# lipku/LiveTalking

Measured on NVIDIA H100. Metric: lip-sync frames/sec (wav2lip256, 256x256, batch 16, mel + U-Net fwd + paste-back), higher is better.
Workload: dtype f16 (fp32 accumulate); mel f64; paste u8

## Files before the change

livetalking_b200/csrc/conv_halo.cu:

```cuda
#include <cuda.h>

#include <atomic>
#include <mutex>
#include <utility>

#include "conv_halo.h"
#include "ltb_internal.h"
#include "ptx_sm90.cuh"

#ifdef LTB_HALO_DIAG
#include <cstdlib>
#define LTB_DIAG(bit) (p.dbg & (bit))
#else
#define LTB_DIAG(bit) 0
#endif

namespace ltb {

constexpr int kHaloP = 10;
constexpr int kHaloThreads = 384;
constexpr int kProducerRegs = 40, kConsumerRegs = 232;
constexpr int kSms = 132;

template <int BN, int NSUB, int NACC, int TAPS, int RC = 0>
struct HaloCfg {
  static constexpr bool HALO = (TAPS != 1);
  static constexpr bool S2 = (TAPS == 10);
  static constexpr int P = S2 ? 9 : (HALO ? kHaloP : 8);
  static constexpr int HR = S2 ? 16 * NSUB + 1 : (HALO ? 16 * NSUB + 2 : 16 * NSUB);
  static constexpr int TG = (TAPS == 9 || TAPS == 10) ? 3 : (TAPS == 16 ? 4 : 1);
  static constexpr int PLANE_BYTES = (HR * P * 128 + 1023) & ~1023;
  static constexpr int A_BYTES_RAW = (S2 ? 4 : 1) * HR * P * 128;
  static constexpr int A_BYTES = S2 ? 4 * PLANE_BYTES : ((A_BYTES_RAW + 1023) & ~1023);
  static constexpr int B_BYTES = TG * BN * 128;
  static constexpr int BUDGET = 223 * 1024;
  static constexpr int A_STAGES_STREAM = S2 ? 2 : ((BN <= 32) ? 4 : (BN <= 64 ? 3 : (NSUB == 1 ? 3 : 2)));
  static constexpr int A_STAGES_RES = ((BUDGET - RC * TG * B_BYTES) / A_BYTES) > 4 ? 4 : ((BUDGET - RC * TG * B_BYTES) / A_BYTES);
  static constexpr int A_STAGES = RC ? A_STAGES_RES : A_STAGES_STREAM;
  static constexpr bool RES_PREFETCH = (BN == 128 && NSUB == 2 && NACC == 1 && TAPS == 9 && RC == 0);
  static constexpr int RES_BYTES = RES_PREFETCH ? 128 * BN * 2 : 0;
  static constexpr int B_STAGES_MAX = (BUDGET - A_STAGES * A_BYTES - RES_BYTES) / B_BYTES;
  static constexpr int B_STAGES = RC ? RC * TG : (B_STAGES_MAX > 8 ? 8 : B_STAGES_MAX);
  static constexpr bool LAG = RC || B_STAGES >= 2 * TG;
  static constexpr int ACOLS = NACC * BN;
  static constexpr int SMEM_BYTES = A_STAGES * A_BYTES + B_STAGES * B_BYTES + RES_BYTES + 1024;
  static_assert(NSUB * ACOLS <= 256, "register accumulator overflow");
  static_assert(B_STAGES >= 2, "not enough shared memory for the weight ring");
  static_assert(A_STAGES >= 2, "not enough shared memory for the halo ring");
  static_assert(SMEM_BYTES + 3584 <= 227 * 1024, "shared memory overflow (dynamic + static)");
};

struct SubpixelView {
  int stage, view, slot0, brow, nslots;
};
constexpr int subpixel_view(int vy, int vx) { return (vy + 1) * kHaloP + (vx + 1); }
template <int TAPS>
struct SubpixelTable;
template <>
struct SubpixelTable<9> {
  static constexpr int NV = 5;
  static constexpr SubpixelView v[NV] = {{0, 0, 0, 0, 3}, {1, 1, 1, 0, 2}, {1, kHaloP + 1, 2, 2, 1}, {2, 0, 3, 2, 1}, {2, kHaloP, 2, 0, 2}};
};
template <>
struct SubpixelTable<16> {
  static constexpr int NV = 10;
  static constexpr SubpixelView v[NV] = {{0, subpixel_view(0, 0), 0, 0, 4},
                                         {1, subpixel_view(-1, 0), 0, 0, 2},  {1, subpixel_view(0, 1), 1, 2, 2},
                                         {2, subpixel_view(1, 0), 2, 0, 2},   {2, subpixel_view(0, -1), 0, 2, 1}, {2, subpixel_view(0, -1), 3, 3, 1},
                                         {3, subpixel_view(-1, -1), 0, 0, 1}, {3, subpixel_view(-1, 1), 1, 1, 1}, {3, subpixel_view(1, 1), 2, 2, 1},
                                         {3, subpixel_view(1, -1), 3, 3, 1}};
};

template <int BN, int SLOT0, int BROW, int R, size_t... S>
__device__ __forceinline__ void subpixel_slots(float (&acc)[R], uint64_t a, uint32_t b_lo, uint32_t b_hi, std::index_sequence<S...>) {
  (wgmma_ss_at<BN, (SLOT0 + (int)S) * BN>(acc, a, wgmma_lohi(b_lo + (BROW + (uint32_t)S) * BN * 8u, b_hi), 1u), ...);
}

template <int BN, int TAPS, int R, size_t... V>
__device__ __forceinline__ void subpixel_issue(float (&acc)[R], int j, int k, uint32_t a_lo0, uint32_t b_lo0, uint32_t a_hi, uint32_t b_hi,
                                               std::index_sequence<V...>) {
  (
      [&] {
        constexpr SubpixelView g = SubpixelTable<TAPS>::v[V];
        if (j == g.stage)
          subpixel_slots<BN, g.slot0, g.brow>(acc, wgmma_lohi(a_lo0 + g.view * 8u + k * 2u, a_hi), b_lo0 + k * 2u, b_hi,
                                              std::make_index_sequence<g.nslots>{});
      }(),
      ...);
}

__device__ __forceinline__ void quad_transpose(uint32_t (&x)[4], int lane) {
  const bool b2 = lane & 2, b1 = lane & 1;
  uint32_t s0 = __shfl_xor_sync(0xffffffffu, b2 ? x[0] : x[2], 2);
  uint32_t s1 = __shfl_xor_sync(0xffffffffu, b2 ? x[1] : x[3], 2);
  x[0] = b2 ? s0 : x[0];
  x[1] = b2 ? s1 : x[1];
  x[2] = b2 ? x[2] : s0;
  x[3] = b2 ? x[3] : s1;
  s0 = __shfl_xor_sync(0xffffffffu, b1 ? x[0] : x[1], 1);
  s1 = __shfl_xor_sync(0xffffffffu, b1 ? x[2] : x[3], 1);
  x[0] = b1 ? s0 : x[0];
  x[2] = b1 ? s1 : x[2];
  x[1] = b1 ? x[1] : s0;
  x[3] = b1 ? x[3] : s1;
}

constexpr bool halo_res_smem_ok(int BN, int NSUB, int NACC, int TAPS) { return TAPS == 9 && NACC == 1 && BN * NSUB <= 128; }

template <int BN, int NSUB, int NACC, int TAPS, int RC, bool GRP>
__global__ void __launch_bounds__(kHaloThreads, 1) conv_halo_wgmma_kernel(const __grid_constant__ HaloParams p) {
  static_assert(!GRP || TAPS == 1, "grouped weights exist in GEMM mode only");
  using C = HaloCfg<BN, NSUB, NACC, TAPS, RC>;
  extern __shared__ uint8_t smem_raw[];
  __shared__ __align__(8) uint64_t a_full[C::A_STAGES], a_empty[C::A_STAGES];
  __shared__ __align__(8) uint64_t b_full[C::B_STAGES], b_empty[C::B_STAGES];
  __shared__ float head_sw[100];
  constexpr int kGnSmem = (NACC == 1) ? 512 : 1;
  __shared__ float gn_acc[kGnSmem];

  const int tid = threadIdx.x, warp = tid >> 5, lane = tid & 31;
  constexpr bool kHeadOk = (BN == 32 && NACC == 1 && TAPS == 9);
  const bool gn_smem = NACC == 1 && p.gn_stats != nullptr && p.gn_images * p.gn_groups * 2 <= kGnSmem;
  if (gn_smem)
    for (int i = tid; i < p.gn_images * p.gn_groups * 2; i += kHaloThreads) gn_acc[i] = 0.f;
  constexpr bool kHaloMode = C::HALO;
  if (kHeadOk && p.head_out && tid < 99) head_sw[tid] = (tid < 96) ? p.head_w[tid] : p.head_b[tid - 96];
  const uint32_t smem0 = (smem_u32(smem_raw) + 1023u) & ~1023u;
  const uint32_t a_smem = smem0;
  const uint32_t b_smem = smem0 + C::A_STAGES * C::A_BYTES;
  const int chunks = (p.Cin + 63) / 64;

  if (tid == 0) {
    for (int s = 0; s < C::A_STAGES; ++s) {
      mbar_init(smem_u32(&a_full[s]), 1);
      mbar_init(smem_u32(&a_empty[s]), 8);
    }
    for (int s = 0; s < C::B_STAGES; ++s) {
      mbar_init(smem_u32(&b_full[s]), 1);
      mbar_init(smem_u32(&b_empty[s]), 8);
    }
    mbar_fence_init();
    tma_prefetch_desc(&p.tm_in);
    tma_prefetch_desc(&p.tm_w);
  }
  __syncthreads();

  const int tiles_m = kHaloMode ? p.tiles_x * p.tiles_y * p.N : p.tiles_x;

  pdl_launch_dependents();
  if (RC && warp == 8 && lane == 0) {
    mbar_arrive_expect_tx(smem_u32(&b_full[0]), RC * C::TG * C::B_BYTES);
    for (int c = 0; c < RC; ++c)
      for (int j = 0; j < C::TG; ++j)
        tma_load_3d(b_smem + (c * C::TG + j) * C::B_BYTES, &p.tm_w, smem_u32(&b_full[0]), c * 64, 0, j * C::TG);
  }
  pdl_wait();

  if (warp >= 8) {
    setmaxnreg_dec<kProducerRegs>();
    if (warp == 8 && lane == 0) {
      uint32_t ai = 0, bi = 0;
      for (int t = blockIdx.x; t < p.total_tiles; t += gridDim.x) {
        const int nt = t / tiles_m;
        int mt = t - nt * tiles_m;
        int img = 0, y0 = 0, x0 = 0;
        int g_row = 0, g_slot = 0;
        if constexpr (GRP) {
          const int g = mt / p.group_tiles;
          g_row = g * p.group_rows + (mt - g * p.group_tiles) * (128 * NSUB);
          g_slot = p.group_slot[g];
        }
        if (kHaloMode) {
          img = mt / (p.tiles_x * p.tiles_y);
          mt -= img * (p.tiles_x * p.tiles_y);
          const int ty = mt / p.tiles_x, tx = mt - ty * p.tiles_x;
          y0 = ty * (16 * NSUB) + p.halo_y0;
          x0 = tx * 8 + p.halo_x0;
        }
        for (int c = 0; c < chunks; ++c) {
          const uint32_t as = ai % C::A_STAGES;
          mbar_wait(smem_u32(&a_empty[as]), ((ai / C::A_STAGES) & 1u) ^ 1u);
          if (LTB_DIAG(8)) {
            mbar_arrive(smem_u32(&a_full[as]));
          } else {
            mbar_arrive_expect_tx(smem_u32(&a_full[as]), C::A_BYTES_RAW);
            if (C::S2) {
#pragma unroll
              for (int pl = 0; pl < 4; ++pl)
                tma_load_4d(a_smem + as * C::A_BYTES + pl * C::PLANE_BYTES, &p.tm_in, smem_u32(&a_full[as]), c * 64,
                            2 * (x0 + 1) - (pl & 1), 2 * (y0 + 1) - (pl >> 1), img);
            } else if (kHaloMode) tma_load_4d(a_smem + as * C::A_BYTES, &p.tm_in, smem_u32(&a_full[as]), c * 64, x0, y0, img);
            else if constexpr (GRP) tma_load_2d(a_smem + as * C::A_BYTES, &p.tm_in, smem_u32(&a_full[as]), c * 64, g_row);
            else tma_load_2d(a_smem + as * C::A_BYTES, &p.tm_in, smem_u32(&a_full[as]), c * 64, mt * (128 * NSUB));
          }
          ++ai;
          if (RC) continue;
          for (int j = 0; j < C::TG; ++j) {
            const uint32_t bs = bi % C::B_STAGES;
            mbar_wait(smem_u32(&b_empty[bs]), ((bi / C::B_STAGES) & 1u) ^ 1u);
            if (LTB_DIAG(16)) {
              mbar_arrive(smem_u32(&b_full[bs]));
              ++bi;
              continue;
            }
            mbar_arrive_expect_tx(smem_u32(&b_full[bs]), C::B_BYTES);
            if (kHaloMode) tma_load_3d(b_smem + bs * C::B_BYTES, &p.tm_w, smem_u32(&b_full[bs]), c * 64, nt * BN, j * C::TG);
            else if constexpr (GRP) tma_load_3d(b_smem + bs * C::B_BYTES, &p.tm_w, smem_u32(&b_full[bs]), c * 64, nt * BN, g_slot);
            else tma_load_2d(b_smem + bs * C::B_BYTES, &p.tm_w, smem_u32(&b_full[bs]), c * 64, nt * BN);
            ++bi;
          }
        }
      }
    }
  } else {
    setmaxnreg_inc<kConsumerRegs>();
    const int wg = warp >> 2, wq = warp & 3;
    const int cq = 2 * (lane & 3);
    constexpr uint32_t kAHi = wgmma_hi_128b(C::P * 128);
    constexpr uint32_t kBHi = wgmma_hi_128b(1024);
    constexpr uint32_t kRowsPerSub = C::HALO ? 16u * C::P : 128u;
    const uint32_t wg_off = (uint32_t)wg * (C::HALO ? 8u * C::P : 64u) * 8u;
    constexpr bool kResHalo = halo_res_smem_ok(BN, NSUB, NACC, TAPS);
    const int res_row = (8 * wg + 2 * wq + ((lane >> 3) & 1) + 1) * C::P + (lane & 7) + 1;
    const int res_kb = lane >> 4;
    auto halo_pix = [&](int img, int ty, int tx, int sub, int sl, int r, bool& ok) -> size_t {
      const int gy = ty * (16 * NSUB) + sub * 16 + wg * 8 + (r >> 3), gx = tx * 8 + (r & 7);
      ok = gy < p.GH && gx < p.GW;
      return ((size_t)img * p.OH + gy * p.osy + p.acc_oy[sl]) * p.OW + gx * p.osx + p.acc_ox[sl];
    };
    const uint32_t res_buf = b_smem + C::B_STAGES * C::B_BYTES;
    if (RC) mbar_wait(smem_u32(&b_full[0]), 0);
    uint32_t ai = 0, bi = 0;
    for (int t = blockIdx.x; t < p.total_tiles; t += gridDim.x) {
      const int nt = t / tiles_m;
      int mt = t - nt * tiles_m;
      int img = 0, ty = 0, tx = 0;
      if (kHaloMode) {
        img = mt / (p.tiles_x * p.tiles_y);
        mt -= img * (p.tiles_x * p.tiles_y);
        ty = mt / p.tiles_x;
        tx = mt - ty * p.tiles_x;
      }
      const int n0 = nt * BN;
      const bool res_pf = C::RES_PREFETCH && p.res != nullptr && !LTB_DIAG(1);
      auto res_src = [&](int sub, int r, bool& ok) {
        const size_t px = halo_pix(img, ty, tx, sub, 0, r, ok);
        return reinterpret_cast<const uint4*>(p.res + (ok ? px : 0) * p.RCtot + p.rc_off + n0 + 8 * (lane & 3));
      };
      if constexpr (C::RES_PREFETCH) {
        if (res_pf) {
#pragma unroll
          for (int hh = 0; hh < 2; ++hh) {
            bool ok;
            const uint4* src = res_src(0, wq * 16 + (lane >> 2) + 8 * hh, ok);
#pragma unroll
            for (int m = 0; m < BN / 32; ++m) cp_async16(res_buf + ((hh * (BN / 32) + m) * 256 + tid) * 16, src + 4 * m, ok ? 16u : 0u);
          }
          cp_async_commit();
        }
      }
      uint4 rpf[2][BN / 32];
      float acc[NSUB][C::ACOLS / 2];
#pragma unroll
      for (int s = 0; s < NSUB; ++s)
#pragma unroll
        for (int i = 0; i < C::ACOLS / 2; ++i) acc[s][i] = 0.f;
      uint32_t rh[NSUB][2][BN / 8];
      const int n0_res = (t / tiles_m) * BN;
      const int c_res = (kResHalo && p.res_halo) ? n0_res / 64 : chunks;
      const int cb_res = (BN == 32) ? (n0_res & 63) >> 3 : 0;
      uint32_t pend_as = 0, pend_bs = 0;
      bool pend = false;
#pragma unroll 1
      for (int c = 0; c < chunks; ++c) {
        const uint32_t as = ai % C::A_STAGES;
        mbar_wait(smem_u32(&a_full[as]), (ai / C::A_STAGES) & 1u);
        if constexpr (kResHalo) {
          if (c == c_res || (BN == 128 && c == c_res + 1)) {
            const bool hi = BN == 128 && c != c_res;
            const uint32_t rbase = a_smem + as * C::A_BYTES + res_row * 128;
#pragma unroll
            for (int s = 0; s < NSUB; ++s)
#pragma unroll
              for (int i = 0; i < BN / 8; i += 2) {
                if (BN == 128 && (i >= 8) != hi) continue;
                const uint32_t chunk16 = (uint32_t)(((cb_res + i + res_kb) & 7) ^ (res_row & 7));
                ldmatrix_x4(rh[s][0][i], rh[s][1][i], rh[s][0][i + 1], rh[s][1][i + 1], rbase + s * (16 * C::P * 128) + chunk16 * 16);
              }
          }
        }
        const uint32_t a_lo0 = wgmma_lo(a_smem + as * C::A_BYTES) + wg_off;
        const uint32_t bs0 = bi % C::B_STAGES;
#pragma unroll
        for (int j = 0; j < C::TG; ++j) {
          const uint32_t bs = RC ? (uint32_t)(c * C::TG + j) : (bi + j) % C::B_STAGES;
          if (!RC) mbar_wait(smem_u32(&b_full[bs]), ((bi + j) / C::B_STAGES) & 1u);
          const uint32_t b_lo0 = wgmma_lo(b_smem + bs * C::B_BYTES);
          if (!LTB_DIAG(4)) wgmma_fence();
#pragma unroll
          for (int k = 0; k < 4; ++k) {
            if (LTB_DIAG(4)) break;
            if constexpr (NACC == 1) {
#pragma unroll
              for (int tt = 0; tt < C::TG; ++tt) {
                const uint32_t aoff = C::S2 ? (uint32_t)(((j != 1) * 2 + (tt != 1)) * (C::PLANE_BYTES / 16) + ((j == 2) * C::P + (tt == 2)) * 8)
                                            : (kHaloMode ? (uint32_t)(j * C::P + tt) * 8u : 0u);
                const uint64_t bd = wgmma_lohi(b_lo0 + tt * (BN * 8) + k * 2, kBHi);
#pragma unroll
                for (int sub = 0; sub < NSUB; ++sub)
                  Wgmma<BN>::ss(acc[sub], wgmma_lohi(a_lo0 + aoff + sub * kRowsPerSub * 8 + k * 2, kAHi), bd, 1u);
              }
            } else {
              subpixel_issue<BN, TAPS>(acc[0], j, k, a_lo0, b_lo0, kAHi, kBHi, std::make_index_sequence<SubpixelTable<TAPS>::NV>{});
            }
          }
          if constexpr (!C::LAG) {
            wgmma_commit();
            wgmma_wait<0>();
            __syncwarp();
            if (lane == 0) mbar_arrive(smem_u32(&b_empty[bs]));
          }
        }
        if (C::LAG) {
          wgmma_commit();
          wgmma_wait<1>();
          if (pend) {
            __syncwarp();
            if (lane == 0) {
              mbar_arrive(smem_u32(&a_empty[pend_as]));
              if (!RC)
                for (int j = 0; j < C::TG; ++j) mbar_arrive(smem_u32(&b_empty[(pend_bs + j) % C::B_STAGES]));
            }
          }
          pend = true;
          pend_as = as;
          pend_bs = bs0;
        } else {
          __syncwarp();
          if (lane == 0) mbar_arrive(smem_u32(&a_empty[as]));
        }
        ++ai;
        if (!RC) bi += C::TG;
      }
      if constexpr (C::RES_PREFETCH) {
        if (res_pf) {
#pragma unroll
          for (int hh = 0; hh < 2; ++hh) {
            bool ok;
            const uint4* src = res_src(1, wq * 16 + (lane >> 2) + 8 * hh, ok);
#pragma unroll
            for (int m = 0; m < BN / 32; ++m) rpf[hh][m] = ok ? __ldcg(src + 4 * m) : make_uint4(0u, 0u, 0u, 0u);
          }
        }
      }
      wgmma_wait<0>();
      if (C::RES_PREFETCH && res_pf) cp_async_wait<0>();
#pragma unroll
      for (int s = 0; s < NSUB; ++s) wgmma_fence_regs(acc[s]);
      if (C::LAG && pend) {
        __syncwarp();
        if (lane == 0) {
          mbar_arrive(smem_u32(&a_empty[pend_as]));
          if (!RC)
            for (int j = 0; j < C::TG; ++j) mbar_arrive(smem_u32(&b_empty[(pend_bs + j) % C::B_STAGES]));
        }
      }
      if (LTB_DIAG(2)) continue;

      const float* bias = p.bias;
      int g_tile = 0;
      if constexpr (GRP) {
        g_tile = mt / p.group_tiles;
        bias += p.group_slot[g_tile] * p.bias_slot_stride;
      }
      const bool has_res = (p.res != nullptr) && !LTB_DIAG(1);
      const bool res_smem = kResHalo && has_res && p.res_halo;
      const bool res_gmem = has_res && !res_smem;
      const bool head = kHeadOk && p.head_out != nullptr;
      float2 bb[BN / 8];
#pragma unroll
      for (int i = 0; i < BN / 8; ++i) bb[i] = __ldg(reinterpret_cast<const float2*>(bias + n0 + 8 * i + cq));
      const __half2 hmax = __floats2half2_rn(65504.f, 65504.f);
      const __half2 hlo = p.relu ? __floats2half2_rn(0.f, 0.f) : __floats2half2_rn(-65504.f, -65504.f);
      auto add_res = [&](uint32_t v, uint32_t r) {
        const __half2 o = __hmin2(__hmax2(__hadd2(*reinterpret_cast<const __half2*>(&v), *reinterpret_cast<const __half2*>(&r)), hlo), hmax);
        return *reinterpret_cast<const uint32_t*>(&o);
      };
#pragma unroll
      for (int sub = 0; sub < NSUB; ++sub) {
        float gs[BN / 8], gq[BN / 8];
#pragma unroll
        for (int i = 0; i < BN / 8; ++i) gs[i] = gq[i] = 0.f;
#pragma unroll
        for (int sl = 0; sl < NACC; ++sl) {
#pragma unroll
          for (int hh = 0; hh < 2; ++hh) {
// ... 134 lines not shown
  std::call_once(once, []() {
    void* p = nullptr;
    cudaDriverEntryPointQueryResult q;
    if (cudaGetDriverEntryPoint("cuTensorMapEncodeTiled", &p, cudaEnableDefault, &q) == cudaSuccess &&
        q == cudaDriverEntryPointSuccess)
      fn = reinterpret_cast<EncodeTiledFn>(p);
  });
  return fn;
}

static bool encode(CUtensorMap* tm, int rank, const void* base, const cuuint64_t* dims, const cuuint64_t* strides_bytes,
                   const cuuint32_t* box, int spatial_stride = 1) {
  EncodeTiledFn fn = get_encode();
  if (!fn) return false;
  cuuint32_t es[5] = {1, (cuuint32_t)spatial_stride, (cuuint32_t)spatial_stride, 1, 1};
  return fn(tm, CU_TENSOR_MAP_DATA_TYPE_FLOAT16, (cuuint32_t)rank, const_cast<void*>(base), dims, strides_bytes, box, es,
            CU_TENSOR_MAP_INTERLEAVE_NONE, CU_TENSOR_MAP_SWIZZLE_128B, CU_TENSOR_MAP_L2_PROMOTION_L2_256B,
            CU_TENSOR_MAP_FLOAT_OOB_FILL_NONE) == CUDA_SUCCESS;
}

static bool is_conv3x3(const ConvParams& p) {
  if (p.nphases != 1 || p.ph[0].ntaps != 9 || p.sy != 1 || p.sx != 1 || p.osy != 1 || p.osx != 1) return false;
  for (int t = 0; t < 9; ++t)
    if (p.ph[0].dy[t] != t / 3 - 1 || p.ph[0].dx[t] != t % 3 - 1) return false;
  return p.IH == p.GH && p.IW == p.GW && p.OH == p.GH && p.OW == p.GW;
}
static bool is_convT(const ConvParams& p) {
  if (p.nphases != 4 || p.osy != 2 || p.osx != 2 || p.sy != 1 || p.sx != 1) return false;
  const int nt[4] = {1, 2, 2, 4};
  for (int i = 0; i < 4; ++i)
    if (p.ph[i].ntaps != nt[i]) return false;
  return p.IH == p.GH && p.IW == p.GW && p.OH == 2 * p.GH && p.OW == 2 * p.GW;
}

static bool is_conv3x3_s2(const ConvParams& p) {
  if (p.nphases != 1 || p.ph[0].ntaps != 9 || p.sy != 2 || p.sx != 2 || p.osy != 1 || p.osx != 1) return false;
  for (int t = 0; t < 9; ++t)
    if (p.ph[0].dy[t] != t / 3 - 1 || p.ph[0].dx[t] != t % 3 - 1) return false;
  return p.IH == 2 * p.GH && p.IW == 2 * p.GW && p.OH == p.GH && p.OW == p.GW;
}

static bool is_upconv(const ConvParams& p) {
  return p.upconv == 1 && p.nphases == 4 && p.osy == 2 && p.osx == 2 && p.sy == 1 && p.sx == 1 && p.IH == p.GH && p.IW == p.GW &&
         p.OH == 2 * p.GH && p.OW == 2 * p.GW;
}

static bool is_gemm(const ConvParams& p) {
  return p.nphases == 1 && p.ph[0].ntaps == 1 && p.ph[0].dy[0] == 0 && p.ph[0].dx[0] == 0 && p.sy == 1 && p.sx == 1 && p.osy == 1 &&
         p.osx == 1 && p.IH == p.GH && p.IW == p.GW && p.OH == p.GH && p.OW == p.GW;
}

static bool pick_cfg(const ConvParams& p, int* BN, int* NSUB, int* NACC);

bool conv_halo_supported(const ConvParams& p) {
  if (p.zbatch > 1) return false;
  if ((p.OCtot % 8) || (p.oc_off % 8) || (reinterpret_cast<uintptr_t>(p.out) % 16)) return false;
  if (p.res && ((p.RCtot % 8) || (p.rc_off % 8) || (reinterpret_cast<uintptr_t>(p.res) % 16))) return false;
  if (p.group_slot && (!is_gemm(p) || (p.w_slot_stride * 2) % 16 != 0)) return false;
  if (is_gemm(p)) {
    return p.Cout % 32 == 0 && p.Cin % 8 == 0 && p.Cin >= 32 && (p.ICtot % 8) == 0 && (p.ic_off % 8) == 0 && (p.Ktot % 8) == 0 &&
           (p.ph[0].koff % 8) == 0 && p.M >= 512 && get_encode() != nullptr;
  }
  if (is_conv3x3_s2(p)) {
    return p.Cout % 32 == 0 && p.Cin >= 64 && (p.ICtot % 8) == 0 && (p.ic_off % 8) == 0 && p.Ktot == 9 * p.Cin && p.GH >= 16 &&
           p.GW >= 8 && get_encode() != nullptr;
  }
  if (is_upconv(p))
    return p.Cout % 64 == 0 && p.Cin >= 16 && (p.ICtot % 8) == 0 && (p.ic_off % 8) == 0 && p.Ktot == 16 * p.Cin && get_encode() != nullptr;
  if (!(is_conv3x3(p) || is_convT(p))) return false;
  if (p.Cout % 32 != 0 || p.Cin < 16) return false;
  if ((p.ICtot % 8) || (p.ic_off % 8) || (p.Ktot != 9 * p.Cin)) return false;
  if (p.GH % 16 != 0 || p.GW % 8 != 0) {
    int BN, NSUB, NACC;
    if (!pick_cfg(p, &BN, &NSUB, &NACC)) return false;
    const long tiles = (long)p.N * ((p.GH + 16 * NSUB - 1) / (16 * NSUB)) * ((p.GW + 7) / 8) * (p.Cout / BN);
    const long waves = (tiles + kSms - 1) / kSms, chunks = (p.Cin + 63) / 64;
    if (waves * chunks > 16) return false;
  }
  return get_encode() != nullptr;
}

static bool pick_cfg(const ConvParams& p, int* BN, int* NSUB, int* NACC) {
  if (is_gemm(p)) {
    *NACC = 1;
    *BN = (p.Cout % 128 == 0) ? 128 : (p.Cout % 64 == 0) ? 64 : 32;
    auto tiles = [&](int bn, int nsub) { return (long)((p.M + 128 * nsub - 1) / (128 * nsub)) * (p.Cout / bn); };
    *NSUB = tiles(*BN, 2) >= kSms ? 2 : 1;
    while (*BN > 32 && tiles(*BN, *NSUB) < kSms - kSms / 8) *BN >>= 1;
    if (*BN == 128) *NSUB = 1;
    return true;
  }
  if (is_upconv(p)) {
    *NACC = 4;
    *NSUB = 1;
    *BN = 64;
    return true;
  }
  if (is_conv3x3_s2(p)) {
    *NACC = 1;
    *NSUB = 1;
    *BN = (p.Cout % 64 == 0) ? 64 : 32;
    return true;
  }
  const bool tr = is_convT(p);
  *NACC = tr ? 4 : 1;
  if (tr) {
    *NSUB = 1;
    *BN = (p.Cout % 64 == 0) ? 64 : 32;
    return true;
  }
  const long ksteps = (p.Cin + 15) / 16;
  double best = 1e30;
  for (int bn : {128, 64, 32}) {
    if (p.Cout % bn) continue;
    for (int nsub : {2, 1}) {
      if (nsub == 2 && (p.GH % 32) != 0) continue;
      const long tiles = (long)p.N * ((p.GH + 16 * nsub - 1) / (16 * nsub)) * ((p.GW + 7) / 8) * (p.Cout / bn);
      const long waves = (tiles + kSms - 1) / kSms;
      const double tile = (double)ksteps * 9 * nsub * (55.0 + 0.2 * bn) + 800.0;
      const double epi = (waves == 1) ? 40.0 * nsub * bn : 0.0;
      const double cost = waves * tile + epi;
      if (cost < best * 0.9) {
        best = cost;
        *BN = bn;
        *NSUB = nsub;
      }
    }
  }
  return best < 1e30;
}

int conv_halo_make_plan(const ConvParams& p, const __half* w_tap_major, HaloPlan* out) {
  if (!conv_halo_supported(p)) return 1;
  HaloParams& h = out->hp;
  std::memset(&h, 0, sizeof(h));
  out->grouped = false;
  int BN, NSUB, NACC;
  if (!pick_cfg(p, &BN, &NSUB, &NACC)) return 1;
  out->BN = BN;
  out->NSUB = NSUB;
  out->NACC = NACC;
  const bool up = is_upconv(p);
  const bool s2 = is_conv3x3_s2(p);
  const bool tr = NACC == 4 && !up;
  const bool gemm = is_gemm(p);
  out->TAPS = gemm ? 1 : (up ? 16 : (s2 ? 10 : 9));
  if (gemm) {
    cuuint64_t dims[2] = {(cuuint64_t)p.Cin, (cuuint64_t)p.M};
    cuuint64_t strides[1] = {(cuuint64_t)p.ICtot * 2};
    cuuint32_t box[2] = {64, (cuuint32_t)(128 * NSUB)};
    if (!encode(&h.tm_in, 2, p.in + p.ic_off, dims, strides, box)) return 2;
    cuuint64_t wdims[3] = {(cuuint64_t)p.Cin, (cuuint64_t)p.Cout, (cuuint64_t)p.slots};
    cuuint64_t wstrides[2] = {(cuuint64_t)p.Ktot * 2, (cuuint64_t)p.w_slot_stride * 2};
    cuuint32_t wbox[3] = {64, (cuuint32_t)BN, 1};
    if (!encode(&h.tm_w, p.group_slot ? 3 : 2, p.w + p.ph[0].koff, wdims, wstrides, wbox)) return 2;
  } else
  {
    cuuint64_t dims[4] = {(cuuint64_t)p.Cin, (cuuint64_t)p.IW, (cuuint64_t)p.IH, (cuuint64_t)p.N};
    cuuint64_t strides[3] = {(cuuint64_t)p.ICtot * 2, (cuuint64_t)p.IW * p.ICtot * 2, (cuuint64_t)p.IH * p.IW * p.ICtot * 2};
    cuuint32_t box[4] = {64, (cuuint32_t)kHaloP, (cuuint32_t)(16 * NSUB + 2), 1};
    if (s2) {
      box[1] = 2 * 9 - 1;
      box[2] = 2 * (16 * NSUB + 1) - 1;
    }
    if (!encode(&h.tm_in, 4, p.in + p.ic_off, dims, strides, box, s2 ? 2 : 1)) return 2;
  }
  if (up) {
    cuuint64_t dims[3] = {(cuuint64_t)p.Cin, (cuuint64_t)p.Cout, 16};
    cuuint64_t strides[2] = {(cuuint64_t)p.Cin * 2, (cuuint64_t)p.Cout * p.Cin * 2};
    cuuint32_t box[3] = {64, (cuuint32_t)BN, 4};
    if (!encode(&h.tm_w, 3, w_tap_major, dims, strides, box)) return 2;
  } else if (!gemm) {
    cuuint64_t dims[3] = {(cuuint64_t)p.Cin, (cuuint64_t)p.Cout, 9};
    cuuint64_t strides[2] = {(cuuint64_t)p.Cin * 2, (cuuint64_t)p.Cout * p.Cin * 2};
    cuuint32_t box[3] = {64, (cuuint32_t)BN, 3};
    if (!encode(&h.tm_w, 3, w_tap_major, dims, strides, box)) return 2;
  }
  h.out = p.out;
  h.res = p.res;
  h.bias = p.bias;
  h.N = p.N;
  h.M = p.M;
  h.Cin = p.Cin;
  h.gn_stats = nullptr;
#ifdef LTB_HALO_DIAG
  if (const char* e = std::getenv("LTB_HALO_DIAG")) h.dbg = std::atoi(e);
#endif
  h.OCtot = p.OCtot;
  h.oc_off = p.oc_off;
  h.RCtot = p.RCtot;
  h.rc_off = p.rc_off;
  h.OH = p.OH;
  h.OW = p.OW;
  h.GH = p.GH;
  h.GW = p.GW;
  h.osy = p.osy;
  h.osx = p.osx;
  h.relu = p.relu;
  h.res_halo = halo_res_smem_ok(BN, NSUB, NACC, out->TAPS) && p.res != nullptr && p.res == p.in && p.Cin == p.Cout &&
               p.rc_off == p.ic_off && p.RCtot == p.ICtot;
  h.halo_y0 = tr ? 0 : -1;
  h.halo_x0 = tr ? 0 : -1;
  if (up || tr) {
    const int slot_phase[4] = {0, 1, 3, 2};
    for (int sl = 0; sl < 4; ++sl) {
      h.acc_oy[sl] = p.ph[slot_phase[sl]].ooy;
      h.acc_ox[sl] = p.ph[slot_phase[sl]].oox;
    }
  } else {
    h.acc_oy[0] = p.ph[0].ooy;
    h.acc_ox[0] = p.ph[0].oox;
  }
  h.tiles_n = p.Cout / BN;
  if (gemm) {
    h.halo_y0 = h.halo_x0 = 0;
    h.tiles_x = (p.M + 128 * NSUB - 1) / (128 * NSUB);
    if (p.group_slot) {
      out->grouped = true;
      h.group_slot = p.group_slot;
      h.group_rows = p.group_images * p.GH * p.GW;
      h.group_tiles = (h.group_rows + 128 * NSUB - 1) / (128 * NSUB);
      h.bias_slot_stride = p.bias_slot_stride;
      h.tiles_x = (p.N / p.group_images) * h.group_tiles;
    }
    h.tiles_y = 1;
    h.total_tiles = h.tiles_x * h.tiles_n;
    return 0;
  }
  h.tiles_x = (p.GW + 7) / 8;
  h.tiles_y = (p.GH + 16 * NSUB - 1) / (16 * NSUB);
  h.total_tiles = h.tiles_x * h.tiles_y * p.N * h.tiles_n;
  return 0;
}

template <int BN, int NSUB, int NACC, int TAPS = 9, int RC = 0, bool GRP = false>
static cudaError_t launch_cfg(const HaloPlan& pl, int sms, cudaStream_t st) {
  using C = HaloCfg<BN, NSUB, NACC, TAPS, RC>;
  static SmemConfigOnce once;
  if (cudaError_t e = once.ensure(conv_halo_wgmma_kernel<BN, NSUB, NACC, TAPS, RC, GRP>, C::SMEM_BYTES); e != cudaSuccess) return e;
  const int grid = pl.hp.total_tiles < sms ? pl.hp.total_tiles : sms;
  return launch_kernel_pdl(conv_halo_wgmma_kernel<BN, NSUB, NACC, TAPS, RC, GRP>, dim3(grid), dim3(kHaloThreads), C::SMEM_BYTES, st, pl.hp);
}

int conv_halo_sms() {
  static std::atomic<int> sms_cached{0};
  int sms = sms_cached.load();
  if (!sms) {
    int dev = 0;
    cudaGetDevice(&dev);
    cudaDeviceGetAttribute(&sms, cudaDevAttrMultiProcessorCount, dev);
    if (sms <= 0) sms = kSms;
    sms_cached.store(sms);
  }
  return sms;
}

int conv_halo_resident_chunks(const HaloPlan& pl, int sms) {
  if (pl.TAPS != 9 || pl.hp.tiles_n != 1 || pl.hp.total_tiles < 2 * sms) return 0;
  const int key = pl.BN * 100 + pl.NSUB * 10 + pl.NACC;
  const int chunks = (pl.hp.Cin + 63) / 64;
  if (chunks == 1 && (key == 6421 || key == 3221 || key == 6414 || key == 3214)) return 1;
  if (chunks == 2 && (key == 3221 || key == 6414 || key == 3214)) return 2;
  return 0;
}

cudaError_t launch_conv_halo(const HaloPlan& pl, cudaStream_t st) {
  const int sms = conv_halo_sms();
  if (pl.TAPS == 10) {
    if (pl.NSUB != 1 || pl.NACC != 1) return cudaErrorInvalidValue;
    return pl.BN == 64 ? launch_cfg<64, 1, 1, 10>(pl, sms, st) : (pl.BN == 32 ? launch_cfg<32, 1, 1, 10>(pl, sms, st) : cudaErrorInvalidValue);
  }
  if (pl.TAPS == 16) return (pl.BN == 64 && pl.NSUB == 1 && pl.NACC == 4) ? launch_cfg<64, 1, 4, 16>(pl, sms, st) : cudaErrorInvalidValue;
  const int key = pl.BN * 100 + pl.NSUB * 10 + pl.NACC;
  if (pl.TAPS == 1 && pl.grouped) {
    switch (key) {
      case 12811: return launch_cfg<128, 1, 1, 1, 0, true>(pl, sms, st);
      case 6421: return launch_cfg<64, 2, 1, 1, 0, true>(pl, sms, st);
      case 6411: return launch_cfg<64, 1, 1, 1, 0, true>(pl, sms, st);
      case 3221: return launch_cfg<32, 2, 1, 1, 0, true>(pl, sms, st);
      case 3211: return launch_cfg<32, 1, 1, 1, 0, true>(pl, sms, st);
    }
    return cudaErrorInvalidValue;
  }
  if (pl.TAPS == 1) {
    switch (key) {
      case 12811: return launch_cfg<128, 1, 1, 1>(pl, sms, st);
      case 6421: return launch_cfg<64, 2, 1, 1>(pl, sms, st);
      case 6411: return launch_cfg<64, 1, 1, 1>(pl, sms, st);
      case 3221: return launch_cfg<32, 2, 1, 1>(pl, sms, st);
      case 3211: return launch_cfg<32, 1, 1, 1>(pl, sms, st);
    }
    return cudaErrorInvalidValue;
  }
  switch (conv_halo_resident_chunks(pl, sms) * 100000 + key) {
    case 106421: return launch_cfg<64, 2, 1, 9, 1>(pl, sms, st);
    case 103221: return launch_cfg<32, 2, 1, 9, 1>(pl, sms, st);
    case 203221: return launch_cfg<32, 2, 1, 9, 2>(pl, sms, st);
    case 206414: return launch_cfg<64, 1, 4, 9, 2>(pl, sms, st);
    case 106414: return launch_cfg<64, 1, 4, 9, 1>(pl, sms, st);
    case 103214: return launch_cfg<32, 1, 4, 9, 1>(pl, sms, st);
    case 203214: return launch_cfg<32, 1, 4, 9, 2>(pl, sms, st);
  }
  switch (key) {
    case 12821: return launch_cfg<128, 2, 1>(pl, sms, st);
    case 12811: return launch_cfg<128, 1, 1>(pl, sms, st);
    case 6421: return launch_cfg<64, 2, 1>(pl, sms, st);
    case 6411: return launch_cfg<64, 1, 1>(pl, sms, st);
    case 3221: return launch_cfg<32, 2, 1>(pl, sms, st);
    case 3211: return launch_cfg<32, 1, 1>(pl, sms, st);
    case 6414: return launch_cfg<64, 1, 4>(pl, sms, st);
    case 3214: return launch_cfg<32, 1, 4>(pl, sms, st);
  }
  return cudaErrorInvalidValue;
}

bool conv_halo_gn_fusable(const HaloPlan& pl, int cout_total, int groups, int hw) {
  if (pl.NACC != 1 || groups <= 0 || cout_total % groups) return false;
  const int cpg = cout_total / groups;
  if (cpg < 4 || (cpg & (cpg - 1))) return false;
  if (pl.TAPS == 1 && (hw % 128) != 0) return false;
  return true;
}

__global__ void w_tap_major_kernel(const __half* __restrict__ w, __half* __restrict__ wt, int cout, int cin, int ntaps) {
  const size_t i = (size_t)blockIdx.x * blockDim.x + threadIdx.x;
  const size_t total = (size_t)cout * ntaps * cin;
  if (i >= total) return;
  const int ci = (int)(i % cin);
  const int tap = (int)((i / cin) % ntaps);
  const int co = (int)(i / ((size_t)cin * ntaps));
  wt[((size_t)tap * cout + co) * cin + ci] = w[i];
}

cudaError_t launch_w_tap_major(const __half* w, __half* wt, int cout, int cin, cudaStream_t st, int ntaps) {
  const size_t total = (size_t)cout * ntaps * cin;
  w_tap_major_kernel<<<(unsigned)((total + 255) / 256), 256, 0, st>>>(w, wt, cout, cin, ntaps);
  return cudaGetLastError();
}

__global__ void w_tap_major_convT_kernel(const __half* __restrict__ w, __half* __restrict__ wt, int cout, int cin) {
  const size_t i = (size_t)blockIdx.x * blockDim.x + threadIdx.x;
  const size_t total = (size_t)cout * 9 * cin;
  if (i >= total) return;
  const int ci = (int)(i % cin);
  const int tap = (int)((i / cin) % 9);
  const int co = (int)(i / ((size_t)cin * 9));
  const int pos_of_old[9] = {0, 1, 3, 8, 7, 2, 4, 6, 5};
// ... 11 lines not shown
```

livetalking_b200/csrc/conv_halo.h:

```cpp
#pragma once
#include <cuda.h>
#include <cuda_runtime.h>

#include <cstring>

#include "conv_params.h"

namespace ltb {

struct alignas(64) HaloParams {
  CUtensorMap tm_in;
  CUtensorMap tm_w;
  __half* out;
  const __half* res;
  const float* bias;
  int N, M, Cin;
  int OCtot, oc_off, RCtot, rc_off;
  int OH, OW, osy, osx;
  int GH, GW;
  int relu;
  int res_halo;
  int halo_y0, halo_x0;
  int acc_oy[4], acc_ox[4];
  int tiles_x, tiles_y, tiles_n, total_tiles;
  float* gn_stats;
  int gn_groups, gn_cpg, gn_hw, gn_images;
  const float* head_w;
  const float* head_b;
  float* head_out;
  const int* group_slot;
  int group_rows, group_tiles;
  long long bias_slot_stride;
#ifdef LTB_HALO_DIAG
  int dbg;
#endif
};

struct HaloPlan {
  HaloParams hp;
  int BN, NSUB, NACC, TAPS;
  bool grouped;
};

bool conv_halo_supported(const ConvParams& p);
int conv_halo_make_plan(const ConvParams& p, const __half* w_tap_major, HaloPlan* out);
cudaError_t launch_conv_halo(const HaloPlan& pl, cudaStream_t st);
int conv_halo_sms();
int conv_halo_resident_chunks(const HaloPlan& pl, int sms);
bool conv_halo_gn_fusable(const HaloPlan& pl, int cout_total, int groups, int hw);
cudaError_t launch_w_tap_major(const __half* w, __half* wt, int cout, int cin, cudaStream_t st, int ntaps = 9);
cudaError_t launch_w_tap_major_convT(const __half* w, __half* wt, int cout, int cin, cudaStream_t st);

}
```

livetalking_b200/csrc/conv_plan.cu:

```cuda
#include <cstring>
#include <string>
#include <vector>

#include "../../include/ltb200.h"
#include "conv_plan.h"
#include "ltb_internal.h"

namespace ltb {

static const int kTd[2][2] = {{0, 0}, {0, 1}};
static const int kTk[2][2] = {{1, 0}, {2, 0}};
static const int kTn[2] = {1, 2};
static const int kUd[2][2] = {{-1, 0}, {0, 1}};

ConvParams conv_params(ConvMode mode, int N, ConvSlice in, int IH, int IW, int Cin, ConvSlice out, int OH, int OW, int Cout,
                       ConvSlice res, const __half* w, int Ktot, int w_koff, const float* bias, bool relu, ConvTaps taps) {
  ConvParams p;
  std::memset(&p, 0, sizeof(p));
  p.in = in.p;
  p.N = N;
  p.IH = IH;
  p.IW = IW;
  p.ICtot = in.Ctot;
  p.ic_off = in.off;
// ... 39 lines not shown
      for (int b = 0; b < 2; ++b) {
        ConvPhase& ph = p.ph[a * 2 + b];
        const int na = up ? 2 : kTn[a], nb = up ? 2 : kTn[b];
        ph.ntaps = na * nb;
        ph.koff = koff;
        ph.ooy = a;
        ph.oox = b;
        for (int i = 0; i < na; ++i)
          for (int j = 0; j < nb; ++j) {
            ph.dy[i * nb + j] = (signed char)(up ? kUd[a][i] : kTd[a][i]);
            ph.dx[i * nb + j] = (signed char)(up ? kUd[b][j] : kTd[b][j]);
          }
        koff += ph.ntaps * Cin;
      }
  }
  p.M = N * p.GH * p.GW;
  return p;
}

int conv_plan(const ConvParams& p, const __half* w_tap, ConvPath path, ConvPlan* out) {
  out->p = p;
  out->halo = false;
  if (p.group_slot) {
    if (p.group_images < 1 || p.N % p.group_images || p.slots < 1 || p.w_slot_stride < 0 || p.bias_slot_stride < 0)
      return LTB_FAIL("conv: grouped weights need N divisible by group_images >= 1, slots >= 1 and non-negative slot strides");
    if (p.zbatch > 1 || p.upconv) return LTB_FAIL("conv: grouped weights cannot be combined with zbatch or the fused upsample");
  }
  if (path == ConvPath::Gather) return 0;
  const bool gemm = p.nphases == 1 && p.ph[0].ntaps == 1;
  if (!((w_tap || gemm) && conv_halo_supported(p))) {
    if (path == ConvPath::Auto) return 0;
    return LTB_FAIL("conv: the halo kernel cannot run " + std::to_string(p.N) + "x" + std::to_string(p.IH) + "x" + std::to_string(p.IW) +
                    "x" + std::to_string(p.Cin) + " -> " + std::to_string(p.OH) + "x" + std::to_string(p.OW) + "x" + std::to_string(p.Cout) +
                    (w_tap || gemm ? "" : " without tap-major weights"));
  }
  if (conv_halo_make_plan(p, w_tap, &out->hp) != 0) return LTB_FAIL("conv: halo plan / tensor map creation failed");
  out->halo = true;
  return 0;
}

cudaError_t conv_launch(const ConvPlan& pl, cudaStream_t st, float* splitk_ws, size_t ws_floats) {
  return pl.halo ? launch_conv_halo(pl.hp, st) : launch_conv_gather(pl.p, st, splitk_ws, ws_floats);
}

bool conv_plan_variant(const ConvPlan& pl, bool have_ws, size_t ws_floats, ltb_conv_variant* out) {
  std::memset(out, 0, sizeof(*out));
  out->grouped = pl.p.group_slot != nullptr;
  if (pl.halo) {
    out->kernel = 1;
    out->taps = pl.hp.TAPS;
    out->bn = pl.hp.BN;
    out->nsub = pl.hp.NSUB;
    out->nacc = pl.hp.NACC;
    out->resident_chunks = conv_halo_resident_chunks(pl.hp, conv_halo_sms());
    out->res_halo = pl.hp.hp.res_halo;
    return true;
  }
  int ksplit = 0;
  if (!conv_gather_pick(pl.p, have_ws, ws_floats, &out->bn, &out->kb, &ksplit)) return false;
  out->ksplit = ksplit > 1 ? ksplit : 1;
  return true;
}

bool conv_plan_fuse_gn_stats(ConvPlan* pl, float* stats, int groups, int hw) {
  const ConvParams& p = pl->p;
  if (!pl->halo || pl->hp.grouped || p.oc_off != 0 || p.OCtot != p.Cout || !conv_halo_gn_fusable(pl->hp, p.Cout, groups, hw)) return false;
  HaloParams& h = pl->hp.hp;
  h.gn_stats = stats;
  h.gn_groups = groups;
  h.gn_cpg = p.Cout / groups;
  h.gn_hw = hw;
  h.gn_images = p.M / hw;
  return true;
}

bool conv_plan_fuse_head(ConvPlan* pl, const float* w, const float* b, float* out) {
  if (!pl->halo || pl->hp.grouped || pl->hp.BN != 32 || pl->p.Cout != 32) return false;
  pl->hp.hp.head_w = w;
  pl->hp.hp.head_b = b;
  pl->hp.hp.head_out = out;
  return true;
}

static void pack_conv_w(const float* w, int cout, int cin, int KH, int KW, std::vector<__half>& out) {
  out.resize((size_t)cout * KH * KW * cin);
  for (int co = 0; co < cout; ++co)
    for (int kh = 0; kh < KH; ++kh)
      for (int kw = 0; kw < KW; ++kw)
        for (int ci = 0; ci < cin; ++ci)
          out[((size_t)co * KH * KW + kh * KW + kw) * cin + ci] = __float2half(w[(((size_t)co * cin + ci) * KH + kh) * KW + kw]);
}
static void pack_convT_w(const float* w, int cin, int cout, std::vector<__half>& out) {
  out.resize((size_t)cout * 9 * cin);
  for (int co = 0; co < cout; ++co) {
    size_t k = 0;
    for (int a = 0; a < 2; ++a)
      for (int b = 0; b < 2; ++b)
        for (int i = 0; i < kTn[a]; ++i)
          for (int j = 0; j < kTn[b]; ++j) {
            const int kh = kTk[a][i], kw = kTk[b][j];
            for (int ci = 0; ci < cin; ++ci, ++k)
              out[(size_t)co * 9 * cin + k] = __float2half(w[(((size_t)ci * cout + co) * 3 + kh) * 3 + kw]);
          }
  }
}

}
// ... 113 lines not shown
```

livetalking_b200/csrc/ptx_sm90.cuh:

```cuda
#pragma once
#include <cuda_fp16.h>
#include <cstdint>
#include <cstdio>

namespace ltb {

__device__ __forceinline__ uint32_t smem_u32(const void* p) {
  return static_cast<uint32_t>(__cvta_generic_to_shared(p));
}

__device__ __forceinline__ void mbar_init(uint32_t bar, uint32_t count) {
  asm volatile("mbarrier.init.shared::cta.b64 [%0], %1;" ::"r"(bar), "r"(count) : "memory");
}
__device__ __forceinline__ void mbar_fence_init() {
  asm volatile("fence.mbarrier_init.release.cluster;" ::: "memory");
}
__device__ __forceinline__ void mbar_arrive(uint32_t bar) {
  asm volatile("mbarrier.arrive.shared::cta.b64 _, [%0];" ::"r"(bar) : "memory");
}
__device__ __forceinline__ void mbar_arrive_expect_tx(uint32_t bar, uint32_t bytes) {
  asm volatile("mbarrier.arrive.expect_tx.shared::cta.b64 _, [%0], %1;" ::"r"(bar), "r"(bytes) : "memory");
}
__device__ __forceinline__ bool mbar_try_wait(uint32_t bar, uint32_t parity) {
  uint32_t ok;
  asm volatile(
      "{\n\t.reg .pred p;\n\t"
      "mbarrier.try_wait.parity.shared::cta.b64 p, [%1], %2;\n\t"
      "selp.u32 %0, 1, 0, p;\n\t}"
      : "=r"(ok)
      : "r"(bar), "r"(parity)
      : "memory");
  return ok != 0;
}
__device__ __forceinline__ void mbar_wait(uint32_t bar, uint32_t parity) {
  if (mbar_try_wait(bar, parity)) return;
  const long long t0 = clock64();
  while (!mbar_try_wait(bar, parity)) {
    if (clock64() - t0 > 8000000000LL) __trap();
  }
}

__device__ __forceinline__ void fence_proxy_async_smem() {
  asm volatile("fence.proxy.async.shared::cta;" ::: "memory");
}

__device__ __forceinline__ void cp_async16(uint32_t dst, const void* src, uint32_t src_bytes) {
  asm volatile("cp.async.cg.shared.global [%0], [%1], 16, %2;" ::"r"(dst), "l"(src), "r"(src_bytes) : "memory");
}
__device__ __forceinline__ void cp_async_commit() { asm volatile("cp.async.commit_group;" ::: "memory"); }
template <int N>
__device__ __forceinline__ void cp_async_wait() {
  asm volatile("cp.async.wait_group %0;" ::"n"(N) : "memory");
}
__device__ __forceinline__ uint4 lds128(uint32_t addr) {
  uint4 v;
  asm volatile("ld.shared.v4.u32 {%0, %1, %2, %3}, [%4];" : "=r"(v.x), "=r"(v.y), "=r"(v.z), "=r"(v.w) : "r"(addr) : "memory");
  return v;
}

__device__ __forceinline__ void tma_prefetch_desc(const void* tmap) {
  asm volatile("prefetch.tensormap [%0];" ::"l"(tmap) : "memory");
}
__device__ __forceinline__ void tma_load_2d(uint32_t dst, const void* tmap, uint32_t bar, int c0, int c1) {
  asm volatile(
      "cp.async.bulk.tensor.2d.shared::cluster.global.mbarrier::complete_tx::bytes [%0], [%1, {%3, %4}], [%2];" ::"r"(dst),
      "l"(tmap), "r"(bar), "r"(c0), "r"(c1)
      : "memory");
}
__device__ __forceinline__ void tma_load_3d(uint32_t dst, const void* tmap, uint32_t bar, int c0, int c1, int c2) {
  asm volatile(
      "cp.async.bulk.tensor.3d.shared::cluster.global.mbarrier::complete_tx::bytes [%0], [%1, {%3, %4, %5}], [%2];" ::"r"(dst),
      "l"(tmap), "r"(bar), "r"(c0), "r"(c1), "r"(c2)
      : "memory");
}
__device__ __forceinline__ void tma_load_4d(uint32_t dst, const void* tmap, uint32_t bar, int c0, int c1, int c2, int c3) {
  asm volatile(
      "cp.async.bulk.tensor.4d.shared::cluster.global.mbarrier::complete_tx::bytes [%0], [%1, {%3, %4, %5, %6}], [%2];" ::"r"(
          dst),
      "l"(tmap), "r"(bar), "r"(c0), "r"(c1), "r"(c2), "r"(c3)
      : "memory");
}
__device__ __forceinline__ void tma_load_5d(uint32_t dst, const void* tmap, uint32_t bar, int c0, int c1, int c2, int c3,
                                            int c4) {
  asm volatile(
      "cp.async.bulk.tensor.5d.shared::cluster.global.mbarrier::complete_tx::bytes [%0], [%1, {%3, %4, %5, %6, %7}], [%2];" ::
          "r"(dst),
      "l"(tmap), "r"(bar), "r"(c0), "r"(c1), "r"(c2), "r"(c3), "r"(c4)
      : "memory");
}

__device__ __forceinline__ void ldmatrix_x4(uint32_t& r0, uint32_t& r1, uint32_t& r2, uint32_t& r3, uint32_t saddr) {
  asm volatile("ldmatrix.sync.aligned.m8n8.x4.shared.b16 {%0, %1, %2, %3}, [%4];"
// ... 218 lines not shown
```

Measured before the change: 6679.

## Ping-pong consumer warpgroups over half-height tiles in resident-weight halo conv

For resident-weight 3x3 halo convs with a single accumulator, each consumer warpgroup now takes its own half-height tile (8 rows per sub-tile) and the two warpgroups alternate tiles. Named barriers pass a turn token between them so one group's epilogue can overlap the other's WGMMA mainloop. The A ring gets up to 8 stages and the empty barrier expects 4 arrivals. The resident-chunk decision moves into plan creation so the TMA box and tile counts match the new tile height. This doubles the tile count and adds per-tile barrier synchronisation, and any error in the ordering could deadlock the kernel.

```diff
diff --git a/livetalking_b200/csrc/conv_halo.cu b/livetalking_b200/csrc/conv_halo.cu
--- a/livetalking_b200/csrc/conv_halo.cu
+++ b/livetalking_b200/csrc/conv_halo.cu
@@ -26,8 +26,11 @@
 struct HaloCfg {
   static constexpr bool HALO = (TAPS != 1);
   static constexpr bool S2 = (TAPS == 10);
+  static constexpr bool PP = RC > 0 && NACC == 1;
+  static constexpr int TH = PP ? 8 * NSUB : 16 * NSUB;
+  static constexpr int SUB_ROWS = PP ? 8 : 16;
   static constexpr int P = S2 ? 9 : (HALO ? kHaloP : 8);
-  static constexpr int HR = S2 ? 16 * NSUB + 1 : (HALO ? 16 * NSUB + 2 : 16 * NSUB);
+  static constexpr int HR = S2 ? 16 * NSUB + 1 : (HALO ? TH + 2 : 16 * NSUB);
   static constexpr int TG = (TAPS == 9 || TAPS == 10) ? 3 : (TAPS == 16 ? 4 : 1);
   static constexpr int PLANE_BYTES = (HR * P * 128 + 1023) & ~1023;
   static constexpr int A_BYTES_RAW = (S2 ? 4 : 1) * HR * P * 128;
@@ -35,7 +38,9 @@
   static constexpr int B_BYTES = TG * BN * 128;
   static constexpr int BUDGET = 223 * 1024;
   static constexpr int A_STAGES_STREAM = S2 ? 2 : ((BN <= 32) ? 4 : (BN <= 64 ? 3 : (NSUB == 1 ? 3 : 2)));
-  static constexpr int A_STAGES_RES = ((BUDGET - RC * TG * B_BYTES) / A_BYTES) > 4 ? 4 : ((BUDGET - RC * TG * B_BYTES) / A_BYTES);
+  static constexpr int A_STAGES_RES_CAP = PP ? 8 : 4;
+  static constexpr int A_STAGES_RES = ((BUDGET - RC * TG * B_BYTES) / A_BYTES) > A_STAGES_RES_CAP ? A_STAGES_RES_CAP
+                                                                                                 : ((BUDGET - RC * TG * B_BYTES) / A_BYTES);
   static constexpr int A_STAGES = RC ? A_STAGES_RES : A_STAGES_STREAM;
   static constexpr bool RES_PREFETCH = (BN == 128 && NSUB == 2 && NACC == 1 && TAPS == 9 && RC == 0);
   static constexpr int RES_BYTES = RES_PREFETCH ? 128 * BN * 2 : 0;
@@ -133,7 +138,7 @@
   if (tid == 0) {
     for (int s = 0; s < C::A_STAGES; ++s) {
       mbar_init(smem_u32(&a_full[s]), 1);
-      mbar_init(smem_u32(&a_empty[s]), 8);
+      mbar_init(smem_u32(&a_empty[s]), C::PP ? 4 : 8);
     }
     for (int s = 0; s < C::B_STAGES; ++s) {
       mbar_init(smem_u32(&b_full[s]), 1);
@@ -174,7 +179,7 @@
           img = mt / (p.tiles_x * p.tiles_y);
           mt -= img * (p.tiles_x * p.tiles_y);
           const int ty = mt / p.tiles_x, tx = mt - ty * p.tiles_x;
-          y0 = ty * (16 * NSUB) + p.halo_y0;
+          y0 = ty * C::TH + p.halo_y0;
           x0 = tx * 8 + p.halo_x0;
         }
         for (int c = 0; c < chunks; ++c) {
@@ -218,20 +223,22 @@
     const int cq = 2 * (lane & 3);
     constexpr uint32_t kAHi = wgmma_hi_128b(C::P * 128);
     constexpr uint32_t kBHi = wgmma_hi_128b(1024);
-    constexpr uint32_t kRowsPerSub = C::HALO ? 16u * C::P : 128u;
-    const uint32_t wg_off = (uint32_t)wg * (C::HALO ? 8u * C::P : 64u) * 8u;
+    constexpr uint32_t kRowsPerSub = C::HALO ? (uint32_t)C::SUB_ROWS * C::P : 128u;
+    const int wg_row = C::PP ? 0 : 8 * wg;
+    const uint32_t wg_off = C::HALO ? (uint32_t)wg_row * C::P * 8u : (uint32_t)wg * 64u * 8u;
     constexpr bool kResHalo = halo_res_smem_ok(BN, NSUB, NACC, TAPS);
-    const int res_row = (8 * wg + 2 * wq + ((lane >> 3) & 1) + 1) * C::P + (lane & 7) + 1;
+    const int res_row = (wg_row + 2 * wq + ((lane >> 3) & 1) + 1) * C::P + (lane & 7) + 1;
     const int res_kb = lane >> 4;
     auto halo_pix = [&](int img, int ty, int tx, int sub, int sl, int r, bool& ok) -> size_t {
-      const int gy = ty * (16 * NSUB) + sub * 16 + wg * 8 + (r >> 3), gx = tx * 8 + (r & 7);
+      const int gy = ty * C::TH + sub * C::SUB_ROWS + wg_row + (r >> 3), gx = tx * 8 + (r & 7);
       ok = gy < p.GH && gx < p.GW;
       return ((size_t)img * p.OH + gy * p.osy + p.acc_oy[sl]) * p.OW + gx * p.osx + p.acc_ox[sl];
     };
     const uint32_t res_buf = b_smem + C::B_STAGES * C::B_BYTES;
     if (RC) mbar_wait(smem_u32(&b_full[0]), 0);
-    uint32_t ai = 0, bi = 0;
-    for (int t = blockIdx.x; t < p.total_tiles; t += gridDim.x) {
+    const int t_step = C::PP ? 2 * gridDim.x : gridDim.x;
+    uint32_t ai = C::PP ? wg * chunks : 0, bi = 0;
+    for (int t = blockIdx.x + (C::PP ? wg * gridDim.x : 0); t < p.total_tiles; t += t_step, ai += C::PP ? chunks : 0) {
       const int nt = t / tiles_m;
       int mt = t - nt * tiles_m;
       int img = 0, ty = 0, tx = 0;
@@ -271,6 +278,7 @@
       const int cb_res = (BN == 32) ? (n0_res & 63) >> 3 : 0;
       uint32_t pend_as = 0, pend_bs = 0;
       bool pend = false;
+      if (C::PP && t != (int)blockIdx.x) bar_sync(1 + wg, 256);
 #pragma unroll 1
       for (int c = 0; c < chunks; ++c) {
         const uint32_t as = ai % C::A_STAGES;
@@ -285,7 +293,7 @@
               for (int i = 0; i < BN / 8; i += 2) {
                 if (BN == 128 && (i >= 8) != hi) continue;
                 const uint32_t chunk16 = (uint32_t)(((cb_res + i + res_kb) & 7) ^ (res_row & 7));
-                ldmatrix_x4(rh[s][0][i], rh[s][1][i], rh[s][0][i + 1], rh[s][1][i + 1], rbase + s * (16 * C::P * 128) + chunk16 * 16);
+                ldmatrix_x4(rh[s][0][i], rh[s][1][i], rh[s][0][i + 1], rh[s][1][i + 1], rbase + s * (kRowsPerSub * 128) + chunk16 * 16);
               }
           }
         }
@@ -342,6 +350,7 @@
         ++ai;
         if (!RC) bi += C::TG;
       }
+      if (C::PP && t + (int)gridDim.x < p.total_tiles) bar_arrive(2 - wg, 256);
       if constexpr (C::RES_PREFETCH) {
         if (res_pf) {
 #pragma unroll
@@ -582,6 +591,17 @@
 
 static bool pick_cfg(const ConvParams& p, int* BN, int* NSUB, int* NACC);
 
+static int resident_chunks(const ConvParams& p, const HaloPlan& pl, int sms) {
+  if (pl.TAPS != 9 || p.Cout != pl.BN) return 0;
+  const long tiles = (long)p.N * ((p.GH + 16 * pl.NSUB - 1) / (16 * pl.NSUB)) * ((p.GW + 7) / 8);
+  if (tiles < 2L * sms) return 0;
+  const int key = pl.BN * 100 + pl.NSUB * 10 + pl.NACC;
+  const int chunks = (p.Cin + 63) / 64;
+  if (chunks == 1 && (key == 6421 || key == 3221 || key == 6414 || key == 3214)) return 1;
+  if (chunks == 2 && (key == 3221 || key == 6414 || key == 3214)) return 2;
+  return 0;
+}
+
 bool conv_halo_supported(const ConvParams& p) {
   if (p.zbatch > 1) return false;
   if ((p.OCtot % 8) || (p.oc_off % 8) || (reinterpret_cast<uintptr_t>(p.out) % 16)) return false;
@@ -675,6 +695,8 @@
   const bool tr = NACC == 4 && !up;
   const bool gemm = is_gemm(p);
   out->TAPS = gemm ? 1 : (up ? 16 : (s2 ? 10 : 9));
+  out->RC = gemm ? 0 : resident_chunks(p, *out, conv_halo_sms());
+  const int tile_rows = (out->RC && NACC == 1) ? 8 * NSUB : 16 * NSUB;
   if (gemm) {
     cuuint64_t dims[2] = {(cuuint64_t)p.Cin, (cuuint64_t)p.M};
     cuuint64_t strides[1] = {(cuuint64_t)p.ICtot * 2};
@@ -688,7 +710,7 @@
   {
     cuuint64_t dims[4] = {(cuuint64_t)p.Cin, (cuuint64_t)p.IW, (cuuint64_t)p.IH, (cuuint64_t)p.N};
     cuuint64_t strides[3] = {(cuuint64_t)p.ICtot * 2, (cuuint64_t)p.IW * p.ICtot * 2, (cuuint64_t)p.IH * p.IW * p.ICtot * 2};
-    cuuint32_t box[4] = {64, (cuuint32_t)kHaloP, (cuuint32_t)(16 * NSUB + 2), 1};
+    cuuint32_t box[4] = {64, (cuuint32_t)kHaloP, (cuuint32_t)(tile_rows + 2), 1};
     if (s2) {
       box[1] = 2 * 9 - 1;
       box[2] = 2 * (16 * NSUB + 1) - 1;
@@ -758,7 +780,7 @@
     return 0;
   }
   h.tiles_x = (p.GW + 7) / 8;
-  h.tiles_y = (p.GH + 16 * NSUB - 1) / (16 * NSUB);
+  h.tiles_y = (p.GH + tile_rows - 1) / tile_rows;
   h.total_tiles = h.tiles_x * h.tiles_y * p.N * h.tiles_n;
   return 0;
 }
@@ -785,15 +807,6 @@
   return sms;
 }
 
-int conv_halo_resident_chunks(const HaloPlan& pl, int sms) {
-  if (pl.TAPS != 9 || pl.hp.tiles_n != 1 || pl.hp.total_tiles < 2 * sms) return 0;
-  const int key = pl.BN * 100 + pl.NSUB * 10 + pl.NACC;
-  const int chunks = (pl.hp.Cin + 63) / 64;
-  if (chunks == 1 && (key == 6421 || key == 3221 || key == 6414 || key == 3214)) return 1;
-  if (chunks == 2 && (key == 3221 || key == 6414 || key == 3214)) return 2;
-  return 0;
-}
-
 cudaError_t launch_conv_halo(const HaloPlan& pl, cudaStream_t st) {
   const int sms = conv_halo_sms();
   if (pl.TAPS == 10) {
@@ -822,7 +835,7 @@
     }
     return cudaErrorInvalidValue;
   }
-  switch (conv_halo_resident_chunks(pl, sms) * 100000 + key) {
+  switch (pl.RC * 100000 + key) {
     case 106421: return launch_cfg<64, 2, 1, 9, 1>(pl, sms, st);
     case 103221: return launch_cfg<32, 2, 1, 9, 1>(pl, sms, st);
     case 203221: return launch_cfg<32, 2, 1, 9, 2>(pl, sms, st);
diff --git a/livetalking_b200/csrc/conv_halo.h b/livetalking_b200/csrc/conv_halo.h
--- a/livetalking_b200/csrc/conv_halo.h
+++ b/livetalking_b200/csrc/conv_halo.h
@@ -39,6 +39,7 @@
 struct HaloPlan {
   HaloParams hp;
   int BN, NSUB, NACC, TAPS;
+  int RC;
   bool grouped;
 };
 
@@ -46,7 +47,6 @@
 int conv_halo_make_plan(const ConvParams& p, const __half* w_tap_major, HaloPlan* out);
 cudaError_t launch_conv_halo(const HaloPlan& pl, cudaStream_t st);
 int conv_halo_sms();
-int conv_halo_resident_chunks(const HaloPlan& pl, int sms);
 bool conv_halo_gn_fusable(const HaloPlan& pl, int cout_total, int groups, int hw);
 cudaError_t launch_w_tap_major(const __half* w, __half* wt, int cout, int cin, cudaStream_t st, int ntaps = 9);
 cudaError_t launch_w_tap_major_convT(const __half* w, __half* wt, int cout, int cin, cudaStream_t st);
diff --git a/livetalking_b200/csrc/conv_plan.cu b/livetalking_b200/csrc/conv_plan.cu
--- a/livetalking_b200/csrc/conv_plan.cu
+++ b/livetalking_b200/csrc/conv_plan.cu
@@ -115,7 +115,7 @@
     out->bn = pl.hp.BN;
     out->nsub = pl.hp.NSUB;
     out->nacc = pl.hp.NACC;
-    out->resident_chunks = conv_halo_resident_chunks(pl.hp, conv_halo_sms());
+    out->resident_chunks = pl.hp.RC;
     out->res_halo = pl.hp.hp.res_halo;
     return true;
   }
diff --git a/livetalking_b200/csrc/ptx_sm90.cuh b/livetalking_b200/csrc/ptx_sm90.cuh
--- a/livetalking_b200/csrc/ptx_sm90.cuh
+++ b/livetalking_b200/csrc/ptx_sm90.cuh
@@ -38,6 +38,13 @@
   while (!mbar_try_wait(bar, parity)) {
     if (clock64() - t0 > 8000000000LL) __trap();
   }
+}
+
+__device__ __forceinline__ void bar_sync(uint32_t id, uint32_t threads) {
+  asm volatile("bar.sync %0, %1;" ::"r"(id), "r"(threads) : "memory");
+}
+__device__ __forceinline__ void bar_arrive(uint32_t id, uint32_t threads) {
+  asm volatile("bar.arrive %0, %1;" ::"r"(id), "r"(threads) : "memory");
 }
 
 __device__ __forceinline__ void fence_proxy_async_smem() {
```

Result: no change. 6717, median of 6 (+0.6%).
